# danpovey/quantization

Measured on AMD Instinct MI355X. Metric: vectors encoded/sec at dim=512, 8 codebooks; uint8 codes bit-exact vs ref, higher is better.
Workload: dtype f32 (products: exact 30-bit fixed point on the i8 MFMA); 1 GPU; Quantizer.encode, dim=512, bytes_per_frame=8, codebook_size=256, refine_indexes_iters=5, batch=65536 fp32 Gaussian vectors per GPU (BASELINE.json configs[1]), seeded synthetic codebooks; global_batch=65536, parallelism=batch-sharded x1, no collective

## Files before the change

quantization_amd/csrc/mcq_fix_kernels.h:

```cpp
#pragma once
#include "mcq_kernels.h"

namespace mcq {

typedef int i32x4 __attribute__((ext_vector_type(4)));
typedef int i32x16 __attribute__((ext_vector_type(16)));

constexpr int kFixTile = 128;
constexpr int kFixColPad = 128;
constexpr int kFixRing = 4;
constexpr int kFixSlot = 32768;
constexpr int kFixOperand = 16384;
constexpr int kFixInfo = kFixRing * kFixSlot;
constexpr int kFixLds = kFixInfo + 4096;
constexpr int kFixLdsScreen = kFixLds + 1024;

__host__ __device__ inline long fix_round_rows(long r) { return (r + kFixTile - 1) / kFixTile * kFixTile; }
__host__ __device__ inline int fix_round_cols(int d) { return (d + kFixColPad - 1) / kFixColPad * kFixColPad; }
__host__ __device__ inline size_t fix_plane_bytes(long R, int D) { return (size_t)fix_round_rows(R) * fix_round_cols(D) * 4; }

__device__ __forceinline__ int fix_q(float v, int e) {
    float s = ldexpf(v, 30 - e);
    s = fminf(fmaxf(s, -1073741824.0f), 1073741824.0f);
    return (int)rintf(s);
// ... 244 lines not shown
    const long MT = g.RA / kFixTile, NT = g.RB / kFixTile;
    const int H = (LOGITS && g.K > kFixTile) ? g.K / kFixTile : 1;
    const long big = g.walk_rows ? NT : MT, small_units = (g.walk_rows ? MT : NT) / H;
    const int xcd = blockIdx.x & 7, slot = blockIdx.x >> 3, per_xcd = gridDim.x >> 3;
    auto tile_of = [&](long t, long &m0, long &n0) -> bool {
        const long unit = t / H, half = t % H;
        const long idx = slot + unit * per_xcd;
        const long bt = (idx / small_units) * 8 + xcd, st = (idx % small_units) * H + half;
        m0 = (g.walk_rows ? st : bt) * kFixTile;
        n0 = (g.walk_rows ? bt : st) * kFixTile;
        return bt < big;
    };
    i32x16 acc[2][NL];
    const int nst = g.Dq / 32;
    const int wu = __builtin_amdgcn_readfirstlane(wave);
    const int op = wu >> 2, chunk = (wu >> 1) & 1, half = wu & 1;
    const long R = op ? g.RB : g.RA;
    const long pl = R * 16, sstride = 8 * R * 16;
    const unsigned dbase = (unsigned)(size_t)smem + op * kFixOperand + (4 * chunk) * 2048 + half * 1024;
    const unsigned voff = lane * 16, voff4 = lane * 4;
    auto base_of = [&](long m0, long n0) { return (op ? g.B + n0 * 16 : g.A + m0 * 16) + (long)(4 * chunk) * R * 16 + half * 1024; };
    auto issue1 = [&](const int8_t *p, int st, int g4) {
        const int8_t *pg = p + g4 * pl;
        const unsigned d = dbase + (st % kFixRing) * kFixSlot + g4 * 2048;
        asm volatile(
            "s_mov_b32 m0, %[d]\n\ts_nop 0\n\t"
            "global_load_lds_dwordx4 %[vo], %[p]\n\t"
            :
            : [vo] "v"(voff), [p] "s"(pg), [d] "s"(d)
            : "memory");
    };
    auto issue_info = [&](long m0, long n0) {
        if (wu < (LOGITS ? 8 : 4)) {
            const void *src = wu < 2 ? static_cast<const void *>(g.ea + m0 + 64 * wu)
                                     : (wu < 4 ? static_cast<const void *>(g.eb + n0 + 64 * (wu - 2))
                                               : (wu < 6 ? static_cast<const void *>(g.bias + m0 + 64 * (wu - 4))
                                                         : static_cast<const void *>(g.wmu + m0 + 64 * (wu - 6))));
            const unsigned d = (unsigned)(size_t)smem + kFixInfo + 256 * (wu < 6 ? wu : wu + 4);
            asm volatile(
                "s_mov_b32 m0, %[d]\n\ts_nop 0\n\t"
                "global_load_lds_dword %[vo], %[p]\n\t"
                :
                : [vo] "v"(voff4), [p] "s"(src), [d] "s"(d)
                : "memory");
        }
    };
    long m0, n0, m0n = 0, n0n = 0;
    if (!tile_of(0, m0, n0)) return;
    const int8_t *pcur = base_of(m0, n0), *pnext = pcur;
    auto step = [&](int st, const i32x4 (&a)[2][NL], const i32x4 (&b)[NL], i32x4 (&an)[2][NL], i32x4 (&bn)[NL]) {
        const char *base = smem + ((st + 1) % kFixRing) * kFixSlot;
        const int8_t *p = (st + 4 < nst) ? pcur + (st + 4) * sstride : pnext + (st + 4 - nst) * sstride;
        constexpr int PI[10] = {0, 0, 1, 0, 1, 2, 0, 1, 2, 3};
        constexpr int PJ[10] = {0, 1, 0, 2, 1, 0, 3, 2, 1, 0};
        constexpr int LO[5] = {0, SCREEN ? 2 : 3, SCREEN ? 4 : 6, SCREEN ? 6 : 8, 10};
#pragma unroll
        for (int g4 = 0; g4 < NL; ++g4) {
            issue1(p, st, g4);
#pragma unroll
            for (int t = 0; t < 2; ++t)
                an[t][g4] = *reinterpret_cast<const i32x4 *>(base + (kh * 4 + g4) * 2048 + (64 * wm + 32 * t + r32) * 16);
            bn[g4] = *reinterpret_cast<const i32x4 *>(base + kFixOperand + (kh * 4 + g4) * 2048 + (32 * wn + r32) * 16);
#pragma unroll
            for (int q = LO[g4]; q < LO[g4 + 1]; ++q)
#pragma unroll
                for (int ta = 0; ta < 2; ++ta)
                    acc[ta][PI[q] + PJ[q]] =
                        __builtin_amdgcn_mfma_i32_32x32x32_i8(a[ta][PI[q]], b[PJ[q]], acc[ta][PI[q] + PJ[q]], 0, 0, 0);
            __builtin_amdgcn_sched_barrier(0);
        }
    };
    i32x4 a0[2][NL], b0[NL], a1[2][NL], b1[NL];
    issue_info(m0, n0);
#pragma unroll
    for (int q = 0; q < 4; ++q)
#pragma unroll
        for (int g4 = 0; g4 < NL; ++g4) issue1(pcur + q * sstride, q, g4);
    if constexpr (SCREEN) asm volatile("s_waitcnt vmcnt(9)" ::: "memory");
    else asm volatile("s_waitcnt vmcnt(12)" ::: "memory");
    __builtin_amdgcn_s_barrier();
#pragma unroll
    for (int l = 0; l < NL; ++l) {
#pragma unroll
        for (int t = 0; t < 2; ++t)
            a0[t][l] = *reinterpret_cast<const i32x4 *>(smem + (kh * 4 + l) * 2048 + (64 * wm + 32 * t + r32) * 16);
        b0[l] = *reinterpret_cast<const i32x4 *>(smem + kFixOperand + (kh * 4 + l) * 2048 + (32 * wn + r32) * 16);
    }
    int *info = reinterpret_cast<int *>(smem + kFixInfo);
    float *infof = reinterpret_cast<float *>(smem + kFixInfo);
    float runv = 0.f;
    int runk = 0;
    float runs = 0.f, runt = 0.f, runq = 0.f;
    int runj = 0, rune = 0;
    for (long t = 0;; ++t) {
        const bool has_next = tile_of(t + 1, m0n, n0n);
        pnext = has_next ? base_of(m0n, n0n) : pcur;
#pragma unroll
        for (int a = 0; a < 2; ++a)
#pragma unroll
            for (int s = 0; s < NL; ++s)
#pragma unroll
                for (int v = 0; v < 16; ++v) acc[a][s][v] = 0;
        for (int st = 0; st < nst; st += 2) {
            if constexpr (SCREEN) asm volatile("s_waitcnt vmcnt(6)\n\ts_waitcnt lgkmcnt(0)" ::: "memory");
            else asm volatile("s_waitcnt vmcnt(8)\n\ts_waitcnt lgkmcnt(0)" ::: "memory");
            __builtin_amdgcn_s_barrier();
            step(st, a0, b0, a1, b1);
            if constexpr (SCREEN) asm volatile("s_waitcnt vmcnt(6)\n\ts_waitcnt lgkmcnt(0)" ::: "memory");
            else asm volatile("s_waitcnt vmcnt(8)\n\ts_waitcnt lgkmcnt(0)" ::: "memory");
            __builtin_amdgcn_s_barrier();
            step(st + 1, a1, b1, a0, b0);
        }
        auto value = [&](int ta, int v, int e) -> float {
            float tt;
            if constexpr (SCREEN) tt = __fmul_rn((float)acc[ta][2][v], 256.0f);
            else tt = __builtin_fmaf((float)acc[ta][2][v], 256.0f, (float)acc[ta][NL - 1][v]);
            tt = __builtin_fmaf((float)acc[ta][1][v], 65536.0f, tt);
            tt = __builtin_fmaf((float)acc[ta][0][v], 16777216.0f, tt);
            return ldexpf(tt, e);
        };
        int rbase = 64 * wm + 4 * kh, cbase = 32 * wn + r32;
        asm volatile("" : "+v"(rbase), "+v"(cbase));
        i32x4 er[2][4];
#pragma unroll
        for (int ta = 0; ta < 2; ++ta)
#pragma unroll
            for (int q = 0; q < 4; ++q) er[ta][q] = *reinterpret_cast<const i32x4 *>(&info[rbase + 32 * ta + 8 * q]);
        const bool full = (m0 + kFixTile <= g.M) && (n0 + kFixTile <= g.N);
        const int ecol = info[128 + cbase] - 36;
        const int rows_left = (int)((g.M - m0 - rbase) > 128 ? 128 : (g.M - m0 - rbase));
        if (MODE == FG_STORE) {
            const bool col_ok = n0 + cbase < g.N;
            float *orow = g.out + (m0 + rbase) * g.ldo + n0 + cbase;
            if (full) {
#pragma unroll
                for (int ta = 0; ta < 2; ++ta)
#pragma unroll
                    for (int v = 0; v < 16; ++v) {
                        const int ro = 32 * ta + 8 * (v >> 2) + (v & 3);
                        orow[(long)ro * g.ldo] = value(ta, v, er[ta][v >> 2][v & 3] + ecol);
                    }
            } else {
#pragma unroll
                for (int ta = 0; ta < 2; ++ta)
#pragma unroll
                    for (int v = 0; v < 16; ++v) {
                        const int ro = 32 * ta + 8 * (v >> 2) + (v & 3);
                        const float val = value(ta, v, er[ta][v >> 2][v & 3] + ecol);
                        if (col_ok && ro < rows_left) orow[(long)ro * g.ldo] = val;
                    }
            }
        } else if constexpr (SCREEN) {
            const float ls = g.lscale_ptr ? *g.lscale_ptr : g.lscale;
            float bv[4], sv[4], tv[4], qm = 0.f;
            int bk[4], sk[4];
            const long col = n0 + cbase;
#pragma unroll
            for (int ta = 0; ta < 2; ++ta) {
#pragma unroll
                for (int v4 = 0; v4 < 4; ++v4) {
                    const f32x4 br4 = *reinterpret_cast<const f32x4 *>(&infof[256 + rbase + 32 * ta + 8 * v4]);
                    const f32x4 wm4 = *reinterpret_cast<const f32x4 *>(&infof[640 + rbase + 32 * ta + 8 * v4]);
#pragma unroll
                    for (int c = 0; c < 4; ++c) {
                        const int v = 4 * v4 + c;
                        const int rl = rbase + 32 * ta + 8 * v4 + c;
                        const float s2 = __fmul_rn(__fadd_rn(value(ta, v, er[ta][v4][c] + ecol), wm4[c]), ls);
                        const float val = __fadd_rn(s2, br4[c]);
                        qm = fmaxf(qm, fmaxf(fabsf(s2), fabsf(val)));
                        const int gi = 2 * ta + (v4 >> 1);
                        if ((v4 & 1) == 0 && c == 0) { bv[gi] = val; bk[gi] = sk[gi] = rl; sv[gi] = tv[gi] = -INFINITY; }
                        else {
                            const bool c1 = val > bv[gi], c2 = val > sv[gi];
                            tv[gi] = __builtin_amdgcn_fmed3f(tv[gi], sv[gi], val);
                            sv[gi] = __builtin_amdgcn_fmed3f(sv[gi], bv[gi], val);
                            sk[gi] = c1 ? bk[gi] : (c2 ? rl : sk[gi]);
                            bk[gi] = c1 ? rl : bk[gi];
                            bv[gi] = fmaxf(bv[gi], val);
                        }
                    }
                }
            }
            int em = info[lane] > info[lane + 64] ? info[lane] : info[lane + 64];
            for (int s = 32; s >= 1; s >>= 1) { const int o = __shfl_xor(em, s, 64); em = o > em ? o : em; }
            auto merge = [](float &b1, int &k1, float &s1, int &j1, float &t1, float b2, int k2, float s2, int j2, float t2) {
                if (b2 > b1) {
                    float f = b1; b1 = b2; b2 = f;
                    f = s1; s1 = s2; s2 = f;
                    t1 = t2;
                    int i = k1; k1 = k2; k2 = i;
                    j1 = j2;
                }
                if (b2 > s1) { t1 = fmaxf(s1, s2); s1 = b2; j1 = k2; }
                else t1 = fmaxf(t1, b2);
            };
            const float cA = 16.5f * 16384.0f * (float)g.Dq;
            auto undecided = [&](float v, float s, float q, int e) {
                const float margin = __fadd_rn(__fadd_rn(__fmul_rn(ldexpf(cA, e + ecol), ls), __fmul_rn(q, 1.9073486328125e-6f)), 7.5231638452626401e-37f);
                return !(__fsub_rn(v, s) > margin);
            };
            auto append = [&](long pos, unsigned second_entry, bool many) {
                const unsigned at = atomicAdd(g.und_cnt, 1u);
                if (at < g.und_cap) {
                    g.und_list[2 * (size_t)at] = (unsigned)pos;
                    g.und_list[2 * (size_t)at + 1] = second_entry | (many ? 0x80000000u : 0u);
                }
            };
            const int K = g.K;
#pragma unroll
            for (int gi = 0; gi < 4; ++gi)
                merge(bv[gi], bk[gi], sv[gi], sk[gi], tv[gi], __shfl_xor(bv[gi], 32, 64), __shfl_xor(bk[gi], 32, 64),
                      __shfl_xor(sv[gi], 32, 64), __shfl_xor(sk[gi], 32, 64), __shfl_xor(tv[gi], 32, 64));
            qm = fmaxf(qm, __shfl_xor(qm, 32, 64));
            if (K >= 32) {
                merge(bv[0], bk[0], sv[0], sk[0], tv[0], bv[1], bk[1], sv[1], sk[1], tv[1]);
                merge(bv[2], bk[2], sv[2], sk[2], tv[2], bv[3], bk[3], sv[3], sk[3], tv[3]);
            }
            if (K >= 64) merge(bv[0], bk[0], sv[0], sk[0], tv[0], bv[2], bk[2], sv[2], sk[2], tv[2]);
            if (K <= 64) {
                if (kh == 0) {
                    const int span = K / 16;
#pragma unroll
                    for (int gi = 0; gi < 4; ++gi) {
                        const long row = m0 + bk[gi];
                        if ((gi % span) == 0 && col < g.N && row < g.M) {
                            fg_store_idx(g, col * g.ncb + row / K, row % K);
                            if (undecided(bv[gi], sv[gi], qm, em))
                                append(col * g.ncb + row / K, (unsigned)((m0 + sk[gi]) % K), undecided(bv[gi], tv[gi], qm, em));
                        }
                    }
                }
            } else {
                float *exv = infof + 384, *exs = infof + 768, *exq = infof + 896;
                int *exk = info + 384 + 128;
                float *ext = reinterpret_cast<float *>(smem + kFixInfo + 4096);
                int *exj = reinterpret_cast<int *>(smem + kFixInfo + 4096 + 512);
                if (wm == 1 && kh == 0) {
                    exv[cbase] = bv[0]; exk[cbase] = bk[0]; exs[cbase] = sv[0]; exq[cbase] = qm;
                    ext[cbase] = tv[0]; exj[cbase] = sk[0];
                }
                asm volatile("s_waitcnt lgkmcnt(0)" ::: "memory");
                __builtin_amdgcn_s_barrier();
                if (wm == 0 && kh == 0) {
                    const int hf = (int)(t % H);
                    float v = bv[0], s = sv[0], t3 = tv[0], q = fmaxf(qm, exq[cbase]);
                    int kk = bk[0], jj = sk[0];
                    merge(v, kk, s, jj, t3, exv[cbase], exk[cbase], exs[cbase], exj[cbase], ext[cbase]);
                    kk += (int)m0;
                    jj += (int)m0;
                    if (hf > 0) {
                        merge(v, kk, s, jj, t3, runv, runk, runs, runj, runt);
                        q = fmaxf(q, runq);
                        em = em > rune ? em : rune;
                    }
                    runv = v; runk = kk; runs = s; runj = jj; runt = t3; runq = q; rune = em;
                    const long k = kk;
                    if (hf == H - 1 && col < g.N && k < g.M) {
                        fg_store_idx(g, col * g.ncb + k / K, k % K);
                        if (undecided(v, s, q, em)) append(col * g.ncb + k / K, (unsigned)(jj % K), undecided(v, t3, q, em));
                    }
                }
            }
        } else {
            const float ls = g.lscale_ptr ? *g.lscale_ptr : g.lscale;
            float bv[4];
            int bk[4];
            const long col = n0 + cbase;
            float *lrow = g.logits ? g.logits + col * g.ldo + m0 + rbase : nullptr;
#pragma unroll
            for (int ta = 0; ta < 2; ++ta) {
#pragma unroll
                for (int v4 = 0; v4 < 4; ++v4) {
                    const f32x4 br4 = *reinterpret_cast<const f32x4 *>(&infof[256 + rbase + 32 * ta + 8 * v4]);
                    const f32x4 wm4 = *reinterpret_cast<const f32x4 *>(&infof[640 + rbase + 32 * ta + 8 * v4]);
                    f32x4 q4;
#pragma unroll
                    for (int c = 0; c < 4; ++c) {
                        const int v = 4 * v4 + c;
                        const int rl = rbase + 32 * ta + 8 * v4 + c;
                        const float val = __fadd_rn(__fmul_rn(__fadd_rn(value(ta, v, er[ta][v4][c] + ecol), wm4[c]), ls), br4[c]);
                        q4[c] = val;
                        const int gi = 2 * ta + (v4 >> 1);
                        if ((v4 & 1) == 0 && c == 0) { bv[gi] = val; bk[gi] = rl; }
                        else if (val > bv[gi]) { bv[gi] = val; bk[gi] = rl; }
                    }
                    if (lrow && (full || (col < g.N && 32 * ta + 8 * v4 < rows_left)))
                        *reinterpret_cast<f32x4 *>(lrow + 32 * ta + 8 * v4) = q4;
                }
            }
            if (g.idx) {
                auto better = [](float v1, int k1, float v2, int k2) { return (v1 > v2) | ((v1 == v2) & (k1 < k2)); };
                const int K = g.K;
#pragma unroll
                for (int gi = 0; gi < 4; ++gi) {
                    const float ov = __shfl_xor(bv[gi], 32, 64);
                    const int ok = __shfl_xor(bk[gi], 32, 64);
                    if (better(ov, ok, bv[gi], bk[gi])) { bv[gi] = ov; bk[gi] = ok; }
                }
                if (K >= 32) {
                    if (bv[1] > bv[0]) { bv[0] = bv[1]; bk[0] = bk[1]; }
                    if (bv[3] > bv[2]) { bv[2] = bv[3]; bk[2] = bk[3]; }
                }
                if (K >= 64 && bv[2] > bv[0]) { bv[0] = bv[2]; bk[0] = bk[2]; }
                if (K <= 64) {
                    if (kh == 0) {
                        const int span = K / 16;
#pragma unroll
                        for (int gi = 0; gi < 4; ++gi) {
                            const long row = m0 + bk[gi];
                            if ((gi % span) == 0 && col < g.N && row < g.M) fg_store_idx(g, col * g.ncb + row / K, row % K);
                        }
                    }
                } else {
                    float *exv = infof + 384;
                    int *exk = info + 384 + 128;
                    if (wm == 1 && kh == 0) { exv[cbase] = bv[0]; exk[cbase] = bk[0]; }
                    asm volatile("s_waitcnt lgkmcnt(0)" ::: "memory");
                    __builtin_amdgcn_s_barrier();
                    if (wm == 0 && kh == 0) {
                        const int hf = (int)(t % H);
                        float v = bv[0];
                        long k = m0 + bk[0];
                        if (better(exv[cbase], exk[cbase], bv[0], bk[0])) { v = exv[cbase]; k = m0 + exk[cbase]; }
                        if (hf > 0 && !(v > runv)) { v = runv; k = runk; }
                        runv = v;
                        runk = (int)k;
                        if (hf == H - 1 && col < g.N && k < g.M) fg_store_idx(g, col * g.ncb + k / K, k % K);
                    }
                }
            }
        }
        if (!has_next) break;
        asm volatile("s_waitcnt lgkmcnt(0)" ::: "memory");
        __builtin_amdgcn_s_barrier();
        m0 = m0n;
        n0 = n0n;
        pcur = pnext;
        issue_info(m0, n0);
    }
    asm volatile("s_waitcnt vmcnt(0)" ::: "memory");
}

struct FixRecheck {
    const int8_t *W, *X;
    const int *ew, *ex;
    long RW, RX;
    int Dq;
    const float *bias, *wmu, *lscale_ptr;
    float lscale;
    void *idx;
    int idx_wide;
    int K, ncb;
    const unsigned *cnt, *list;
    unsigned cap;
};

__global__ void __launch_bounds__(256) k_fscreen_recheck(const FixRecheck a) {
    const int lane = threadIdx.x & 63;
    const unsigned wv = __builtin_amdgcn_readfirstlane(blockIdx.x * 4 + (threadIdx.x >> 6)), nwv = gridDim.x * 4;
    unsigned n = *a.cnt;
    n = n < a.cap ? n : a.cap;
    const float ls = a.lscale_ptr ? *a.lscale_ptr : a.lscale;
    const int K = a.K, nch = a.Dq / 16;
    for (unsigned i = wv; i < n; i += nwv) {
        const unsigned pos = a.list[2 * (size_t)i], snd = a.list[2 * (size_t)i + 1];
        const long col = pos / (unsigned)a.ncb;
        const int cb = (int)(pos % (unsigned)a.ncb);
        const int ecol = a.ex[col] - 36;
        auto chunk = [&](int (&T)[4], int c, long row) {
            i32x4 xl[4], wl[4];
#pragma unroll
            for (int l = 0; l < 4; ++l) {
                xl[l] = *reinterpret_cast<const i32x4 *>(a.X + (((long)c * 4 + l) * a.RX + col) * 16);
                wl[l] = *reinterpret_cast<const i32x4 *>(a.W + (((long)c * 4 + l) * a.RW + row) * 16);
            }
#pragma unroll
            for (int p = 0; p < 4; ++p)
#pragma unroll
                for (int q = 0; p + q < 4; ++q)
#pragma unroll
                    for (int d = 0; d < 4; ++d) T[p + q] = __builtin_amdgcn_sdot4(wl[p][d], xl[q][d], T[p + q], false);
        };
        auto logit = [&](const int (&T)[4], long row) -> float {
            float tt = (float)T[3];
            tt = __builtin_fmaf((float)T[2], 256.0f, tt);
            tt = __builtin_fmaf((float)T[1], 65536.0f, tt);
            tt = __builtin_fmaf((float)T[0], 16777216.0f, tt);
            return __fadd_rn(__fmul_rn(__fadd_rn(ldexpf(tt, a.ew[row] + ecol), a.wmu[row]), ls), a.bias[row]);
        };
        float bv = -INFINITY;
        int bk = 0x7fffffff;
        if ((snd & 0x80000000u) == 0) {
            const int first = a.idx_wide ? (int)static_cast<const uint16_t *>(a.idx)[pos] : (int)static_cast<const uint8_t *>(a.idx)[pos];
            const int j = (lane < 32) ? first : (int)snd;
            const long row = (long)cb * K + j;
            int T[4] = {0, 0, 0, 0};
            for (int c = lane & 31; c < nch; c += 32) chunk(T, c, row);
#pragma unroll
            for (int p = 0; p < 4; ++p)
                for (int sft = 16; sft >= 1; sft >>= 1) T[p] += __shfl_xor(T[p], sft, 64);
            bv = logit(T, row);
            bk = j;
        } else {
            for (int j = lane; j < K; j += 64) {
                const long row = (long)cb * K + j;
                int T[4] = {0, 0, 0, 0};
#pragma unroll 4
                for (int c = 0; c < nch; ++c) chunk(T, c, row);
                const float val = logit(T, row);
                if (j == lane || val > bv) { bv = val; bk = j; }
            }
        }
        for (int s = 32; s >= 1; s >>= 1) {
            const float ov = __shfl_xor(bv, s, 64);
            const int ok = __shfl_xor(bk, s, 64);
            if ((ov > bv) | ((ov == bv) & (ok < bk))) { bv = ov; bk = ok; }
        }
        if (lane == 0) {
            if (a.idx_wide) static_cast<uint16_t *>(a.idx)[pos] = (uint16_t)bk;
            else static_cast<uint8_t *>(a.idx)[pos] = (uint8_t)bk;
        }
    }
}

}
```

quantization_amd/csrc/mcq_kernels.h:

```cpp
#pragma once
#include <hip/hip_runtime.h>
#include <stdint.h>
#include <type_traits>

namespace mcq {

typedef float f32x4 __attribute__((ext_vector_type(4)));

constexpr int kWave = 64;
constexpr int kBigPos = 0x7fffffff;

__device__ __forceinline__ int lane_id() { return threadIdx.x & 63; }

__device__ __forceinline__ float wave_sum_butterfly(float p) {
#pragma unroll
    for (int m = 32; m >= 1; m >>= 1) p = p + __shfl_xor(p, m, 64);
    return p;
}

template <int CTRL>
__device__ __forceinline__ float dpp_f(float x) {
    return __int_as_float(__builtin_amdgcn_update_dpp(0, __float_as_int(x), CTRL, 0xf, 0xf, true));
}
template <int CTRL>
// ... 306 lines not shown
            out_v = __uint_as_float(ev);
            out_p = (int)ep;
            has = lane < cnt;
            dst = lane;
            return cnt;
        }
    }
    u64 key[VPL];
    u64 cmask[VPL];
#pragma unroll
    for (int i = 0; i < VPL; ++i) {
        const bool cand = p[i] != kBigPos;
        key[i] = cand ? (((u64)ord32(v[i]) << 32) | (uint32_t)p[i]) : kKeyMax;
        cmask[i] = __ballot(cand);
    }
    const int target = cnt - 1;
    u64 T = 0;
    for (;;) {
        u64 kp = kKeyMax;
        int ps = -1, pl = 0;
#pragma unroll
        for (int i = VPL - 1; i >= 0; --i)
            if (cmask[i] != 0) { ps = i; pl = __ffsll((long long)cmask[i]) - 1; }
        if (ps < 0) { T = kKeyMax - 1; break; }
#pragma unroll
        for (int i = 0; i < VPL; ++i)
            if (i == ps) kp = readlane_u64(key[i], pl);
        u64 ltm[VPL];
        int r = 0;
#pragma unroll
        for (int i = 0; i < VPL; ++i) {
            ltm[i] = __ballot(key[i] < kp);
            r += __popcll(ltm[i]);
        }
        if (r == target) { T = kp; break; }
#pragma unroll
        for (int i = 0; i < VPL; ++i) {
            const u64 pivot_bit = (i == ps) ? (1ull << pl) : 0ull;
            cmask[i] &= (r > target) ? ltm[i] : ~(ltm[i] | pivot_bit);
        }
    }
    uint32_t *lo = reinterpret_cast<uint32_t *>(lds);
    int d = 0, nsel = 0;
    if constexpr (LAYOUT == kSlotMajor) {
#pragma unroll
        for (int i = 0; i < VPL; ++i) {
            const bool s = key[i] <= T;
            const u64 mi = __ballot(s);
            d = mbcnt64(mi, nsel);
            if (s && d < 64) { lo[d] = __float_as_uint(v[i]); lo[128 + d] = (uint32_t)p[i]; }
            nsel += __popcll(mi);
        }
    } else {
#pragma unroll
        for (int i = 0; i < VPL; ++i) {
            const u64 mi = __ballot(key[i] <= T);
            d = mbcnt64(mi, d);
            nsel += __popcll(mi);
        }
#pragma unroll
        for (int i = 0; i < VPL; ++i) {
            const bool s = key[i] <= T;
            if (s && d < 64) { lo[d] = __float_as_uint(v[i]); lo[128 + d] = (uint32_t)p[i]; }
            d += s ? 1 : 0;
        }
    }
    wave_lds_fence();
    has = lane < nsel;
    const uint32_t ev = lo[lane], ep = lo[128 + lane];
    wave_lds_fence();
    out_v = __uint_as_float(ev);
    out_p = (int)ep;
    dst = lane;
    if constexpr (LAYOUT == kAnyOrder) {
        const int mine = has ? out_p : kBigPos;
        int r = 0;
        for (int j = 0; j < nsel; ++j) r += (__builtin_amdgcn_readlane(mine, j) < mine) ? 1 : 0;
        dst = r;
    }
    return nsel;
}

template <int VPL, int LAYOUT = kLaneMajor>
__global__ void __launch_bounds__(64)
k_test_select(const float *__restrict__ scores, int cnt, float *__restrict__ out_v, int *__restrict__ out_p) {
    __shared__ u64 scratch[kSelectLdsU64];
    const float *sc = scores + (size_t)blockIdx.x * 64 * VPL;
    float v[VPL];
    int p[VPL];
#pragma unroll
    for (int i = 0; i < VPL; ++i) {
        p[i] = (LAYOUT == kSlotMajor) ? 64 * i + lane_id() : VPL * lane_id() + i;
        v[i] = sc[p[i]];
    }
    bool has;
    int dst, op;
    float ov;
    const int nsel = wave_select_set<VPL, LAYOUT>(v, p, cnt, 64 * VPL, scratch, has, dst, ov, op);
    if (has) {
        out_v[(size_t)blockIdx.x * 64 + dst] = ov;
        out_p[(size_t)blockIdx.x * 64 + dst] = op;
    }
    if (lane_id() >= nsel && lane_id() < cnt) {
        out_v[(size_t)blockIdx.x * 64 + lane_id()] = INFINITY;
        out_p[(size_t)blockIdx.x * 64 + lane_id()] = 64 * VPL - 1;
    }
}

__global__ void k_prepare_rows(const float *__restrict__ src, float scale, int apply_scale, long rows, int D,
                               int Dp, float *__restrict__ dst, float *__restrict__ Q,
                               const float *__restrict__ scale_ptr ,
                               float *__restrict__ scales_out ,
                               const float *__restrict__ raw_cs = nullptr, const float *__restrict__ raw_ls = nullptr,
                               float speed = 0.f, float *__restrict__ scales_out2 = nullptr) {
    const long row = (long)blockIdx.x * (blockDim.x >> 6) + (threadIdx.x >> 6);
    if (row >= rows) return;
    const int lane = lane_id();
    if (scale_ptr) {
        scale = *scale_ptr;
        if (scales_out && row == 0 && lane < 2) scales_out[lane] = scale_ptr[lane];
    }
    if (raw_cs) {
        scale = expf(*raw_cs * speed);
        if (row == 0 && lane == 0) {
            const float ls = expf(*raw_ls * speed);
            if (scales_out) { scales_out[0] = scale; scales_out[1] = ls; }
            if (scales_out2) { scales_out2[0] = scale; scales_out2[1] = ls; }
        }
    }
    const float *s = src + row * D;
    float *d = dst + row * Dp;
    float part = 0.f;
    for (int q = lane; q < Dp / 4; q += 64) {
        f32x4 o;
#pragma unroll
        for (int c = 0; c < 4; ++c) {
            const int k = 4 * q + c;
            float val = (k < D) ? s[k] : 0.f;
            if (apply_scale) val = scale * val;
            o[c] = val;
            part = fmaf(val, val, part);
        }
        *reinterpret_cast<f32x4 *>(d + 4 * q) = o;
    }
    part = wave_sum_butterfly(part);
    if (Q != nullptr && lane == 0) Q[row] = part;
}


__global__ void __launch_bounds__(64) k_zero_counts(int *__restrict__ cnt, int n) {
    for (int i = threadIdx.x; i < n; i += blockDim.x) cnt[i] = 0;
}

template <typename CT>
__global__ void k_compact(const CT *__restrict__ idx_old, const CT *__restrict__ idx_new,
                          const int *__restrict__ map_cur, const int *__restrict__ nact, long B, int N, int last,
                          CT *__restrict__ idx_packed, int *__restrict__ map_next, int *__restrict__ cnt_next,
                          const float *__restrict__ E_in, const float *__restrict__ R_in, float *__restrict__ E_out,
                          float *__restrict__ R_out, int pack, uint8_t *__restrict__ out_u8, int64_t *__restrict__ out_i64,
                          uint8_t *__restrict__ codes_also) {
    const long s = (long)blockIdx.x * blockDim.x + threadIdx.x;
    if (nact) B = *nact;
    if (s >= B) return;
    const long orig = map_cur ? (long)map_cur[s] : s;
    bool changed = false;
    if (!last)
        for (int n = 0; n < N; ++n) changed = changed || (idx_old[s * N + n] != idx_new[s * N + n]);
    if (changed) {
        const long slot = atomicAdd(cnt_next, 1);
        for (int n = 0; n < N; ++n) idx_packed[slot * N + n] = idx_new[s * N + n];
        map_next[slot] = (int)orig;
        if (E_in != nullptr) {
            E_out[slot] = E_in[s];
            for (int n = 0; n < N; ++n) R_out[slot * N + n] = R_in[s * N + n];
        }
    } else if (out_i64 != nullptr) {
        for (int n = 0; n < N; ++n) {
            const CT v = idx_new[s * N + n];
            out_i64[orig * N + n] = v;
            if (codes_also) codes_also[orig * N + n] = (uint8_t)v;
        }
    } else if (pack == 1) {
        for (int n = 0; n < N; ++n) out_u8[orig * N + n] = (uint8_t)idx_new[s * N + n];
    } else {
        for (int n = 0; n < N; n += 2) out_u8[orig * (N / 2) + n / 2] = (uint8_t)(idx_new[s * N + n] + 16 * idx_new[s * N + n + 1]);
    }
}

template <typename CT>
__global__ void k_finalize(const CT *__restrict__ idx, long B, int N, int pack, uint8_t *__restrict__ out_u8,
                           int64_t *__restrict__ out_i64, uint8_t *__restrict__ codes_also) {
    const long i = (long)blockIdx.x * blockDim.x + threadIdx.x;
    if (out_i64 != nullptr) {
        if (i < B * N) {
            out_i64[i] = idx[i];
            if (codes_also) codes_also[i] = (uint8_t)idx[i];
        }
    } else {
        const int per = N / pack;
        if (i < B * per) {
            if (pack == 1) out_u8[i] = (uint8_t)idx[i];
            else out_u8[i] = (uint8_t)(idx[2 * i] + 16 * idx[2 * i + 1]);
        }
    }
}

template <typename CT>
__global__ void k_import_indexes(const int64_t *__restrict__ in, long n, int K, CT *__restrict__ out) {
    const long i = (long)blockIdx.x * blockDim.x + threadIdx.x;
    if (i < n) {
        long v = in[i];
        v = v < 0 ? 0 : (v > K - 1 ? K - 1 : v);
        out[i] = (CT)v;
    }
}

template <typename CodeT>
__global__ void k_decode(const CodeT *__restrict__ codes, int per_row, long B, const float *__restrict__ C, int N,
                         int K, int D, int Dp, float *__restrict__ out) {
    const long b = (long)blockIdx.x * (blockDim.x >> 6) + (threadIdx.x >> 6);
    if (b >= B) return;
    const int lane = lane_id();
    const int rep = N / per_row;
    const CodeT *cb = codes + b * per_row;
    float *ob = out + b * D;
    const bool vec_ok = ((D & 3) == 0) && ((reinterpret_cast<uintptr_t>(out) & 15) == 0);
    for (int q = lane; q < Dp / 4; q += 64) {
        f32x4 t = (f32x4){0.f, 0.f, 0.f, 0.f};
        for (int n = 0; n < N; ++n) {
            long code = (long)cb[n / rep];
            int digit = n % rep;
            for (int d = 0; d < digit; ++d) code /= K;
            const int k = (int)(code % K) & (K - 1);
            const f32x4 c = *reinterpret_cast<const f32x4 *>(C + ((long)n * K + k) * Dp + 4 * q);
            t = (n == 0) ? c : t + c;
        }
        if (vec_ok && 4 * q + 3 < D) {
            *reinterpret_cast<f32x4 *>(ob + 4 * q) = t;
        } else {
#pragma unroll
            for (int c = 0; c < 4; ++c)
                if (4 * q + c < D) ob[4 * q + c] = t[c];
        }
    }
}

template <typename CodeT, int CH, int LPV>
__global__ void __launch_bounds__(256)
k_decode_sliced(const CodeT *__restrict__ codes, long B, const float *__restrict__ C, int N, int K, int D, int Dp,
                float *__restrict__ out) {
    constexpr int VPW = 64 / LPV;
    const int slice = blockIdx.x & 7;
    const long vb = blockIdx.x >> 3;
    const int wave = threadIdx.x >> 6, lane = threadIdx.x & 63;
    const int v = lane / LPV, q = lane % LPV;
    const long b = (vb * 4 + wave) * VPW + v;
    const int off = slice * (LPV * 4) + 4 * q;
    if (b >= B || off >= Dp) return;
    const CodeT *cb = codes + b * N;
    const float *Cq = C + off;
    f32x4 t = (f32x4){0.f, 0.f, 0.f, 0.f};
    for (int n0 = 0; n0 < N; n0 += CH) {
        f32x4 rows[CH];
#pragma unroll
        for (int j = 0; j < CH; ++j) {
            const int n = (n0 + j < N) ? n0 + j : N - 1;
            const int k = (int)cb[n] & (K - 1);
            rows[j] = *reinterpret_cast<const f32x4 *>(Cq + ((long)n * K + k) * Dp);
        }
#pragma unroll
        for (int j = 0; j < CH; ++j)
            if (n0 + j < N) t = (n0 + j == 0) ? rows[j] : t + rows[j];
    }
    float *ob = out + b * D + off;
    if (((D & 3) == 0) && ((reinterpret_cast<uintptr_t>(out) & 15) == 0) && off + 3 < D) {
        __builtin_nontemporal_store(t, reinterpret_cast<f32x4 *>(ob));
    } else {
#pragma unroll
        for (int c = 0; c < 4; ++c)
            if (off + c < D) ob[c] = t[c];
    }
}

template <typename CodeT>
__global__ void __launch_bounds__(1024)
k_decode_lds(const CodeT *__restrict__ codes, long B, const float *__restrict__ C, int N, int K, int D, int Dp,
             int groups , float *__restrict__ out) {
    constexpr int W = 16, LPV = W / 4;
    constexpr int UNR = 4;
    extern __shared__ __attribute__((aligned(16))) char smem[];
    f32x4 *rows = reinterpret_cast<f32x4 *>(smem);
    const int ns = Dp / W;
    const int xcd = blockIdx.x & 7, within = blockIdx.x >> 3;
    const int per_xcd = (ns + 7) / 8;
    const int slice = xcd * per_xcd + within % per_xcd;
    const int grp = within / per_xcd;
    if (slice >= ns) return;
    const int tid = threadIdx.x;
    const int nrows = N * K;
    for (int u = tid; u < nrows * LPV; u += blockDim.x)
        rows[u] = *reinterpret_cast<const f32x4 *>(C + (long)(u / LPV) * Dp + slice * W + 4 * (u % LPV));
    __syncthreads();
    const long per = (B + groups - 1) / groups;
    const long b_lo = grp * per, b_hi = (b_lo + per < B) ? b_lo + per : B;
    if (b_lo >= b_hi) return;
    const int q = tid % LPV;
    const int off = slice * W + 4 * q;
    const bool vec_store = ((D & 3) == 0) && ((reinterpret_cast<uintptr_t>(out) & 15) == 0) && off + 3 < D;
    const long stride = blockDim.x / LPV;
    const bool packed = sizeof(CodeT) == 1 && (N == 8 || N == 16) && ((reinterpret_cast<uintptr_t>(codes) & 15) == 0);
    auto fetch = [&](long b, unsigned long long (&w)[2]) {
        const long bc = b < b_hi ? b : b_hi - 1;
        const unsigned long long *p = reinterpret_cast<const unsigned long long *>(reinterpret_cast<const uint8_t *>(codes) + bc * N);
        w[0] = p[0];
        w[1] = (N == 16) ? p[1] : 0ull;
    };
    auto emit = [&](long b, const f32x4 &t) {
        if (b >= b_hi) return;
        float *ob = out + b * D + off;
        if (vec_store) {
            __builtin_nontemporal_store(t, reinterpret_cast<f32x4 *>(ob));
        } else {
#pragma unroll
            for (int c = 0; c < 4; ++c)
                if (off + c < D) ob[c] = t[c];
        }
    };
    if (packed) {
        unsigned long long cur[UNR][2], nxt[UNR][2];
        long b = b_lo + tid / LPV;
#pragma unroll
        for (int u = 0; u < UNR; ++u) fetch(b + u * stride, cur[u]);
        for (; b < b_hi; b += UNR * stride) {
#pragma unroll
            for (int u = 0; u < UNR; ++u) fetch(b + (UNR + u) * stride, nxt[u]);
#pragma unroll
            for (int u = 0; u < UNR; ++u) {
                f32x4 t = rows[((int)(cur[u][0] & 0xffull) & (K - 1)) * LPV + q];
                for (int n = 1; n < N; ++n) {
// ... 204 lines not shown
```

Before: 13.86 million vectors/s.

## Simplify screen top-2 tracking, split recheck by block, vectorize compaction

The screen epilogue stops tracking the runner-up index and third value per lane. The runner-up index is recovered only at the cross-half merge, and any ambiguous case is marked as needing a full recheck. The recheck kernel handles two-candidate entries per wave in a first pass, then spreads full-codebook entries across a whole block with four waves and an LDS reduction instead of using one wave. The compaction kernel uses wave-aggregated atomics and vectorized loads and stores of the code rows when pointers are aligned. The trade-off is that more entries may fall back to the full recheck, and that path now needs block barriers.

After: 13.85 million vectors/s. No clear change (-0.1%).

```diff
diff --git a/quantization_amd/csrc/mcq_fix_kernels.h b/quantization_amd/csrc/mcq_fix_kernels.h
--- a/quantization_amd/csrc/mcq_fix_kernels.h
+++ b/quantization_amd/csrc/mcq_fix_kernels.h
@@ -420,6 +420,7 @@
             }
         } else if constexpr (SCREEN) {
             const float ls = g.lscale_ptr ? *g.lscale_ptr : g.lscale;
+            constexpr int kNoRow = -0x40000000;
             float bv[4], sv[4], tv[4], qm = 0.f;
             int bk[4], sk[4];
             const long col = n0 + cbase;
@@ -434,15 +435,14 @@
                         const int v = 4 * v4 + c;
                         const int rl = rbase + 32 * ta + 8 * v4 + c;
                         const float s2 = __fmul_rn(__fadd_rn(value(ta, v, er[ta][v4][c] + ecol), wm4[c]), ls);
-                        const float val = __fadd_rn(s2, br4[c]);
+                        float val = __fadd_rn(s2, br4[c]);
+                        asm volatile("" : "+v"(val));
                         qm = fmaxf(qm, fmaxf(fabsf(s2), fabsf(val)));
                         const int gi = 2 * ta + (v4 >> 1);
-                        if ((v4 & 1) == 0 && c == 0) { bv[gi] = val; bk[gi] = sk[gi] = rl; sv[gi] = tv[gi] = -INFINITY; }
+                        if ((v4 & 1) == 0 && c == 0) { bv[gi] = val; bk[gi] = rl; sv[gi] = -INFINITY; }
                         else {
-                            const bool c1 = val > bv[gi], c2 = val > sv[gi];
-                            tv[gi] = __builtin_amdgcn_fmed3f(tv[gi], sv[gi], val);
+                            const bool c1 = val > bv[gi];
                             sv[gi] = __builtin_amdgcn_fmed3f(sv[gi], bv[gi], val);
-                            sk[gi] = c1 ? bk[gi] : (c2 ? rl : sk[gi]);
                             bk[gi] = c1 ? rl : bk[gi];
                             bv[gi] = fmaxf(bv[gi], val);
                         }
@@ -476,9 +476,17 @@
             };
             const int K = g.K;
 #pragma unroll
-            for (int gi = 0; gi < 4; ++gi)
-                merge(bv[gi], bk[gi], sv[gi], sk[gi], tv[gi], __shfl_xor(bv[gi], 32, 64), __shfl_xor(bk[gi], 32, 64),
-                      __shfl_xor(sv[gi], 32, 64), __shfl_xor(sk[gi], 32, 64), __shfl_xor(tv[gi], 32, 64));
+            for (int gi = 0; gi < 4; ++gi) {
+                float b2 = __shfl_xor(bv[gi], 32, 64), s2 = __shfl_xor(sv[gi], 32, 64);
+                int k2 = __shfl_xor(bk[gi], 32, 64);
+                if (b2 > bv[gi]) {
+                    float f = bv[gi]; bv[gi] = b2; b2 = f;
+                    f = sv[gi]; sv[gi] = s2; s2 = f;
+                    const int i = bk[gi]; bk[gi] = k2; k2 = i;
+                }
+                if (b2 > sv[gi]) { tv[gi] = fmaxf(sv[gi], s2); sv[gi] = b2; sk[gi] = k2; }
+                else { tv[gi] = sv[gi]; sk[gi] = kNoRow; }
+            }
             qm = fmaxf(qm, __shfl_xor(qm, 32, 64));
             if (K >= 32) {
                 merge(bv[0], bk[0], sv[0], sk[0], tv[0], bv[1], bk[1], sv[1], sk[1], tv[1]);
@@ -494,7 +502,8 @@
                         if ((gi % span) == 0 && col < g.N && row < g.M) {
                             fg_store_idx(g, col * g.ncb + row / K, row % K);
                             if (undecided(bv[gi], sv[gi], qm, em))
-                                append(col * g.ncb + row / K, (unsigned)((m0 + sk[gi]) % K), undecided(bv[gi], tv[gi], qm, em));
+                                append(col * g.ncb + row / K, sk[gi] < 0 ? 0u : (unsigned)((m0 + sk[gi]) % K),
+                                       sk[gi] < 0 || undecided(bv[gi], tv[gi], qm, em));
                         }
                     }
                 }
@@ -525,7 +534,7 @@
                     const long k = kk;
                     if (hf == H - 1 && col < g.N && k < g.M) {
                         fg_store_idx(g, col * g.ncb + k / K, k % K);
-                        if (undecided(v, s, q, em)) append(col * g.ncb + k / K, (unsigned)(jj % K), undecided(v, t3, q, em));
+                        if (undecided(v, s, q, em)) append(col * g.ncb + k / K, jj < 0 ? 0u : (unsigned)(jj % K), jj < 0 || undecided(v, t3, q, em));
                     }
                 }
             }
@@ -624,70 +633,120 @@
 };
 
 __global__ void __launch_bounds__(256) k_fscreen_recheck(const FixRecheck a) {
-    const int lane = threadIdx.x & 63;
-    const unsigned wv = __builtin_amdgcn_readfirstlane(blockIdx.x * 4 + (threadIdx.x >> 6)), nwv = gridDim.x * 4;
+    __shared__ float redv[2][4];
+    __shared__ int redk[2][4];
+    const int lane = threadIdx.x & 63, wave = __builtin_amdgcn_readfirstlane(threadIdx.x >> 6);
+    const unsigned wv = blockIdx.x * 4 + wave, nwv = gridDim.x * 4;
     unsigned n = *a.cnt;
     n = n < a.cap ? n : a.cap;
     const float ls = a.lscale_ptr ? *a.lscale_ptr : a.lscale;
     const int K = a.K, nch = a.Dq / 16;
-    for (unsigned i = wv; i < n; i += nwv) {
-        const unsigned pos = a.list[2 * (size_t)i], snd = a.list[2 * (size_t)i + 1];
-        const long col = pos / (unsigned)a.ncb;
-        const int cb = (int)(pos % (unsigned)a.ncb);
-        const int ecol = a.ex[col] - 36;
-        auto chunk = [&](int (&T)[4], int c, long row) {
-            i32x4 xl[4], wl[4];
-#pragma unroll
-            for (int l = 0; l < 4; ++l) {
-                xl[l] = *reinterpret_cast<const i32x4 *>(a.X + (((long)c * 4 + l) * a.RX + col) * 16);
-                wl[l] = *reinterpret_cast<const i32x4 *>(a.W + (((long)c * 4 + l) * a.RW + row) * 16);
-            }
-#pragma unroll
-            for (int p = 0; p < 4; ++p)
-#pragma unroll
-                for (int q = 0; p + q < 4; ++q)
-#pragma unroll
-                    for (int d = 0; d < 4; ++d) T[p + q] = __builtin_amdgcn_sdot4(wl[p][d], xl[q][d], T[p + q], false);
-        };
-        auto logit = [&](const int (&T)[4], long row) -> float {
-            float tt = (float)T[3];
-            tt = __builtin_fmaf((float)T[2], 256.0f, tt);
-            tt = __builtin_fmaf((float)T[1], 65536.0f, tt);
-            tt = __builtin_fmaf((float)T[0], 16777216.0f, tt);
-            return __fadd_rn(__fmul_rn(__fadd_rn(ldexpf(tt, a.ew[row] + ecol), a.wmu[row]), ls), a.bias[row]);
-        };
-        float bv = -INFINITY;
-        int bk = 0x7fffffff;
-        if ((snd & 0x80000000u) == 0) {
-            const int first = a.idx_wide ? (int)static_cast<const uint16_t *>(a.idx)[pos] : (int)static_cast<const uint8_t *>(a.idx)[pos];
-            const int j = (lane < 32) ? first : (int)snd;
-            const long row = (long)cb * K + j;
-            int T[4] = {0, 0, 0, 0};
-            for (int c = lane & 31; c < nch; c += 32) chunk(T, c, row);
-#pragma unroll
-            for (int p = 0; p < 4; ++p)
-                for (int sft = 16; sft >= 1; sft >>= 1) T[p] += __shfl_xor(T[p], sft, 64);
-            bv = logit(T, row);
-            bk = j;
-        } else {
-            for (int j = lane; j < K; j += 64) {
-                const long row = (long)cb * K + j;
-                int T[4] = {0, 0, 0, 0};
-#pragma unroll 4
-                for (int c = 0; c < nch; ++c) chunk(T, c, row);
-                const float val = logit(T, row);
-                if (j == lane || val > bv) { bv = val; bk = j; }
-            }
-        }
+    long col = 0;
+    int ecol = 0;
+    auto chunk = [&](int (&T)[4], int c, long row) {
+        i32x4 xl[4], wl[4];
+#pragma unroll
+        for (int l = 0; l < 4; ++l) {
+            xl[l] = *reinterpret_cast<const i32x4 *>(a.X + (((long)c * 4 + l) * a.RX + col) * 16);
+            wl[l] = *reinterpret_cast<const i32x4 *>(a.W + (((long)c * 4 + l) * a.RW + row) * 16);
+        }
+#pragma unroll
+        for (int p = 0; p < 4; ++p)
+#pragma unroll
+            for (int q = 0; p + q < 4; ++q)
+#pragma unroll
+                for (int d = 0; d < 4; ++d) T[p + q] = __builtin_amdgcn_sdot4(wl[p][d], xl[q][d], T[p + q], false);
+    };
+    auto logit = [&](const int (&T)[4], long row) -> float {
+        float tt = (float)T[3];
+        tt = __builtin_fmaf((float)T[2], 256.0f, tt);
+        tt = __builtin_fmaf((float)T[1], 65536.0f, tt);
+        tt = __builtin_fmaf((float)T[0], 16777216.0f, tt);
+        return __fadd_rn(__fmul_rn(__fadd_rn(ldexpf(tt, a.ew[row] + ecol), a.wmu[row]), ls), a.bias[row]);
+    };
+    auto wave_first_argmax = [&](float &bv, int &bk) {
         for (int s = 32; s >= 1; s >>= 1) {
             const float ov = __shfl_xor(bv, s, 64);
             const int ok = __shfl_xor(bk, s, 64);
             if ((ov > bv) | ((ov == bv) & (ok < bk))) { bv = ov; bk = ok; }
         }
-        if (lane == 0) {
-            if (a.idx_wide) static_cast<uint16_t *>(a.idx)[pos] = (uint16_t)bk;
-            else static_cast<uint8_t *>(a.idx)[pos] = (uint8_t)bk;
-        }
+    };
+    auto store_code = [&](unsigned pos, int k) {
+        if (a.idx_wide) static_cast<uint16_t *>(a.idx)[pos] = (uint16_t)k;
+        else static_cast<uint8_t *>(a.idx)[pos] = (uint8_t)k;
+    };
+    for (unsigned i = wv; i < n; i += nwv) {
+        const unsigned pos = a.list[2 * (size_t)i], snd = a.list[2 * (size_t)i + 1];
+        if (snd & 0x80000000u) continue;
+        col = pos / (unsigned)a.ncb;
+        const int cb = (int)(pos % (unsigned)a.ncb);
+        ecol = a.ex[col] - 36;
+        const int first = a.idx_wide ? (int)static_cast<const uint16_t *>(a.idx)[pos] : (int)static_cast<const uint8_t *>(a.idx)[pos];
+        const int j = (lane < 32) ? first : (int)snd;
+        const long row = (long)cb * K + j;
+        int T[4] = {0, 0, 0, 0};
+        for (int c = lane & 31; c < nch; c += 32) chunk(T, c, row);
+#pragma unroll
+        for (int p = 0; p < 4; ++p)
+            for (int sft = 16; sft >= 1; sft >>= 1) T[p] += __shfl_xor(T[p], sft, 64);
+        float bv = logit(T, row);
+        int bk = j;
+        wave_first_argmax(bv, bk);
+        if (lane == 0) store_code(pos, bk);
+    }
+    const int rows_per_wave = K / 4;
+    unsigned seen = 0, mine = blockIdx.x, done = 0;
+    auto fetch = [&](unsigned (&w)[8], unsigned i0) {
+#pragma unroll
+        for (int u = 0; u < 8; ++u) {
+            const unsigned i = i0 + 64 * u + lane;
+            w[u] = i < n ? a.list[2 * (size_t)i + 1] : 0u;
+        }
+    };
+    unsigned cur[8], nxt[8];
+    fetch(cur, 0);
+    for (unsigned i0 = 0; i0 < n; i0 += 512) {
+        fetch(nxt, i0 + 512);
+#pragma unroll
+        for (int u = 0; u < 8; ++u) {
+            unsigned long long fl = __ballot((cur[u] >> 31) != 0);
+            while (fl != 0) {
+                const int l = __builtin_ctzll(fl);
+                fl &= fl - 1;
+                if (seen++ != mine) continue;
+                mine += gridDim.x;
+                const unsigned pos = a.list[2 * (size_t)(i0 + 64 * u + l)];
+                col = pos / (unsigned)a.ncb;
+                const int cb = (int)(pos % (unsigned)a.ncb);
+                ecol = a.ex[col] - 36;
+                float bv = -INFINITY;
+                int bk = 0x7fffffff;
+                const int j0 = wave * rows_per_wave + lane;
+                for (int j = j0; j < (wave + 1) * rows_per_wave; j += 64) {
+                    const long row = (long)cb * K + j;
+                    int T[4] = {0, 0, 0, 0};
+#pragma unroll 4
+                    for (int c = 0; c < nch; ++c) chunk(T, c, row);
+                    const float val = logit(T, row);
+                    if (j == j0 || val > bv) { bv = val; bk = j; }
+                }
+                wave_first_argmax(bv, bk);
+                const int buf = done++ & 1;
+                if (lane == 0) { redv[buf][wave] = bv; redk[buf][wave] = bk; }
+                __syncthreads();
+                if (threadIdx.x == 0) {
+#pragma unroll
+                    for (int w = 1; w < 4; ++w) {
+                        const float ov = redv[buf][w];
+                        const int ok = redk[buf][w];
+                        if ((ov > bv) | ((ov == bv) & (ok < bk))) { bv = ov; bk = ok; }
+                    }
+                    store_code(pos, bk);
+                }
+            }
+        }
+#pragma unroll
+        for (int u = 0; u < 8; ++u) cur[u] = nxt[u];
     }
 }
 
diff --git a/quantization_amd/csrc/mcq_kernels.h b/quantization_amd/csrc/mcq_kernels.h
--- a/quantization_amd/csrc/mcq_kernels.h
+++ b/quantization_amd/csrc/mcq_kernels.h
@@ -482,6 +482,125 @@
     for (int i = threadIdx.x; i < n; i += blockDim.x) cnt[i] = 0;
 }
 
+typedef uint32_t cp_u32x2 __attribute__((ext_vector_type(2)));
+typedef uint32_t cp_u32x4 __attribute__((ext_vector_type(4)));
+typedef int64_t cp_i64x2 __attribute__((ext_vector_type(2)));
+
+template <int W>
+__device__ __forceinline__ void cp_load(const void *p, uint32_t (&w)[W / 4]) {
+    if constexpr (W == 4) w[0] = *static_cast<const uint32_t *>(p);
+    else if constexpr (W == 8) {
+        const cp_u32x2 v = *static_cast<const cp_u32x2 *>(p);
+        w[0] = v[0]; w[1] = v[1];
+    } else {
+#pragma unroll
+        for (int q = 0; q < W / 16; ++q) {
+            const cp_u32x4 v = static_cast<const cp_u32x4 *>(p)[q];
+#pragma unroll
+            for (int c = 0; c < 4; ++c) w[4 * q + c] = v[c];
+        }
+    }
+}
+
+template <int NB>
+__device__ __forceinline__ void cp_store(void *p, const uint32_t *w) {
+    if constexpr (NB == 2) *static_cast<uint16_t *>(p) = (uint16_t)w[0];
+    else if constexpr (NB == 4) *static_cast<uint32_t *>(p) = w[0];
+    else if constexpr (NB == 8) *static_cast<cp_u32x2 *>(p) = (cp_u32x2){w[0], w[1]};
+    else {
+#pragma unroll
+        for (int q = 0; q < NB / 16; ++q) static_cast<cp_u32x4 *>(p)[q] = (cp_u32x4){w[4 * q], w[4 * q + 1], w[4 * q + 2], w[4 * q + 3]};
+    }
+}
+
+template <typename CT, int W>
+__device__ __forceinline__ void compact_body(const CT *__restrict__ idx_old, const CT *__restrict__ idx_new,
+                                             const int *__restrict__ map_cur, long B, int N, int last, CT *__restrict__ idx_packed,
+                                             int *__restrict__ map_next, int *__restrict__ cnt_next, const float *__restrict__ E_in,
+                                             const float *__restrict__ R_in, float *__restrict__ E_out, float *__restrict__ R_out,
+                                             int pack, uint8_t *__restrict__ out_u8, int64_t *__restrict__ out_i64,
+                                             uint8_t *__restrict__ codes_also) {
+    constexpr int NWD = W ? W / 4 : 1, NE = W / (int)sizeof(CT);
+    const int lane = lane_id();
+    const long s = (long)blockIdx.x * blockDim.x + threadIdx.x;
+    if (s - lane >= B) return;
+    const bool valid = s < B;
+    const long orig = !valid ? 0 : (map_cur ? (long)map_cur[s] : s);
+    uint32_t wn[NWD];
+    bool changed = false;
+    if (valid) {
+        if constexpr (W != 0) {
+            cp_load<W>(idx_new + s * N, wn);
+            if (!last) {
+                uint32_t wo[NWD], diff = 0;
+                cp_load<W>(idx_old + s * N, wo);
+#pragma unroll
+                for (int q = 0; q < NWD; ++q) diff |= wo[q] ^ wn[q];
+                changed = diff != 0;
+            }
+        } else if (!last) {
+            for (int n = 0; n < N; ++n) changed = changed || (idx_old[s * N + n] != idx_new[s * N + n]);
+        }
+    }
+    const unsigned long long stay = __ballot(changed);
+    if (stay != 0) {
+        int base = 0;
+        if (lane == 0) base = atomicAdd(cnt_next, __popcll(stay));
+        base = __builtin_amdgcn_readfirstlane(base);
+        if (changed) {
+            const long slot = base + (long)__builtin_amdgcn_mbcnt_hi((unsigned)(stay >> 32), __builtin_amdgcn_mbcnt_lo((unsigned)stay, 0u));
+            if constexpr (W != 0) cp_store<W>(idx_packed + slot * N, wn);
+            else
+                for (int n = 0; n < N; ++n) idx_packed[slot * N + n] = idx_new[s * N + n];
+            map_next[slot] = (int)orig;
+            if (E_in != nullptr) {
+                E_out[slot] = E_in[s];
+                if (W != 0 && (N & 3) == 0) {
+                    for (int n = 0; n < N; n += 4)
+                        *reinterpret_cast<f32x4 *>(R_out + slot * N + n) = *reinterpret_cast<const f32x4 *>(R_in + s * N + n);
+                } else {
+                    for (int n = 0; n < N; ++n) R_out[slot * N + n] = R_in[s * N + n];
+                }
+            }
+        }
+    }
+    if (!valid || changed) return;
+    if constexpr (W != 0) {
+        if (out_i64 != nullptr) {
+            constexpr unsigned mask = sizeof(CT) == 1 ? 0xffu : 0xffffu;
+            constexpr int per = 4 / (int)sizeof(CT), bits = 8 * (int)sizeof(CT);
+            cp_i64x2 *o = reinterpret_cast<cp_i64x2 *>(out_i64 + orig * N);
+#pragma unroll
+            for (int n = 0; n < NE; n += 2)
+                o[n / 2] = (cp_i64x2){(int64_t)((wn[n / per] >> (bits * (n % per))) & mask),
+                                      (int64_t)((wn[(n + 1) / per] >> (bits * ((n + 1) % per))) & mask)};
+            if constexpr (sizeof(CT) == 1)
+                if (codes_also) cp_store<W>(codes_also + orig * N, wn);
+        } else if (pack == 1) {
+            if constexpr (sizeof(CT) == 1) cp_store<W>(out_u8 + orig * N, wn);
+        } else if constexpr (sizeof(CT) == 1) {
+            uint32_t pk[(NWD + 1) / 2];
+#pragma unroll
+            for (int q = 0; q < NWD; ++q) {
+                const uint32_t t = wn[q] | (wn[q] >> 4), h = (t & 0xffu) | ((t >> 8) & 0xff00u);
+                if (q & 1) pk[q / 2] |= h << 16;
+                else pk[q / 2] = h;
+            }
+            cp_store<W / 2>(out_u8 + orig * (N / 2), pk);
+        }
+    } else if (out_i64 != nullptr) {
+        for (int n = 0; n < N; ++n) {
+            const CT v = idx_new[s * N + n];
+            out_i64[orig * N + n] = v;
+            if (codes_also) codes_also[orig * N + n] = (uint8_t)v;
+        }
+    } else if (pack == 1) {
+        for (int n = 0; n < N; ++n) out_u8[orig * N + n] = (uint8_t)idx_new[s * N + n];
+    } else {
+        for (int n = 0; n < N; n += 2) out_u8[orig * (N / 2) + n / 2] = (uint8_t)(idx_new[s * N + n] + 16 * idx_new[s * N + n + 1]);
+    }
+}
+
 template <typename CT>
 __global__ void k_compact(const CT *__restrict__ idx_old, const CT *__restrict__ idx_new,
                           const int *__restrict__ map_cur, const int *__restrict__ nact, long B, int N, int last,
@@ -489,32 +608,22 @@
                           const float *__restrict__ E_in, const float *__restrict__ R_in, float *__restrict__ E_out,
                           float *__restrict__ R_out, int pack, uint8_t *__restrict__ out_u8, int64_t *__restrict__ out_i64,
                           uint8_t *__restrict__ codes_also) {
-    const long s = (long)blockIdx.x * blockDim.x + threadIdx.x;
     if (nact) B = *nact;
-    if (s >= B) return;
-    const long orig = map_cur ? (long)map_cur[s] : s;
-    bool changed = false;
-    if (!last)
-        for (int n = 0; n < N; ++n) changed = changed || (idx_old[s * N + n] != idx_new[s * N + n]);
-    if (changed) {
-        const long slot = atomicAdd(cnt_next, 1);
-        for (int n = 0; n < N; ++n) idx_packed[slot * N + n] = idx_new[s * N + n];
-        map_next[slot] = (int)orig;
-        if (E_in != nullptr) {
-            E_out[slot] = E_in[s];
-            for (int n = 0; n < N; ++n) R_out[slot * N + n] = R_in[s * N + n];
-        }
-    } else if (out_i64 != nullptr) {
-        for (int n = 0; n < N; ++n) {
-            const CT v = idx_new[s * N + n];
-            out_i64[orig * N + n] = v;
-            if (codes_also) codes_also[orig * N + n] = (uint8_t)v;
-        }
-    } else if (pack == 1) {
-        for (int n = 0; n < N; ++n) out_u8[orig * N + n] = (uint8_t)idx_new[s * N + n];
-    } else {
-        for (int n = 0; n < N; n += 2) out_u8[orig * (N / 2) + n / 2] = (uint8_t)(idx_new[s * N + n] + 16 * idx_new[s * N + n + 1]);
-    }
+    const uintptr_t ptrs = reinterpret_cast<uintptr_t>(idx_old) | reinterpret_cast<uintptr_t>(idx_new) |
+                           reinterpret_cast<uintptr_t>(idx_packed) | reinterpret_cast<uintptr_t>(out_u8) |
+                           reinterpret_cast<uintptr_t>(out_i64) | reinterpret_cast<uintptr_t>(codes_also);
+    const int W = (ptrs & 15) == 0 ? N * (int)sizeof(CT) : 0;
+#define MCQ_COMPACT_ARGS idx_old, idx_new, map_cur, B, N, last, idx_packed, map_next, cnt_next, E_in, R_in, E_out, R_out, pack, out_u8, out_i64, codes_also
+    switch (W) {
+    case 4: compact_body<CT, 4>(MCQ_COMPACT_ARGS); break;
+    case 8: compact_body<CT, 8>(MCQ_COMPACT_ARGS); break;
+    case 16: compact_body<CT, 16>(MCQ_COMPACT_ARGS); break;
+    case 32: compact_body<CT, 32>(MCQ_COMPACT_ARGS); break;
+    case 64: compact_body<CT, 64>(MCQ_COMPACT_ARGS); break;
+    case 128: compact_body<CT, 128>(MCQ_COMPACT_ARGS); break;
+    default: compact_body<CT, 0>(MCQ_COMPACT_ARGS); break;
+    }
+#undef MCQ_COMPACT_ARGS
 }
 
 template <typename CT>
```
